# KushalChaudhari-16/Medical-Image-Denoising-Using-Diffusion

Measured on AMD Instinct MI355X. Metric: denoised images/sec, 256x256 x50 DDIM steps, higher is better.
Workload: dtype f32 (split-fp16 x3 MFMA, fp32 accumulate); 1 GPU; batch=8/GPU 256x256 grayscale, 50-iteration reverse loop (noise_steps=50, inference_steps=50), random-init 12.8M-param UNet (BASELINE.json configs[1]); batch_per_gpu=8, global_batch=8, parallelism=single, collective=none

## Files before the change

medical-image-denoising-using-diffusion_amd/csrc/conv1x1_f16x3_body.h:

```cpp
#if !defined(MIDD_CONV1_KERNEL) || !defined(MIDD_CONV1_PL)
#error "include from conv1x1_f16x3.hip with MIDD_CONV1_KERNEL and MIDD_CONV1_PL defined"
#endif

template <int MT, int NT, int ATT>
__global__ __launch_bounds__(256, ATT == ATT_PART_IN ? 2 : 3)
void MIDD_CONV1_KERNEL(const ConvArgs a) {
    constexpr int PL = MIDD_CONV1_PL;
    static_assert(PL == 1 || PL == 2, "planes");
    using G = Conv1Geom<MT, NT, PL>;
    constexpr int BM = G::BM, WSTEP = G::WSTEP, WTILE = PL * 1024;
    extern __shared__ __attribute__((aligned(16))) char lds[];

    const int tid = threadIdx.x;
    const int lane = tid & 63;
    const int wave = __builtin_amdgcn_readfirstlane(tid >> 6);
    const int p16 = lane & 15;
    const int kq = lane >> 4;

    const int Cin = a.C0 + a.C1;
    const int csteps = (Cin + 31) >> 5;
    const int nsteps = csteps;
    const int HW = a.OH * a.OW;
    const int tiles = a.tiles_x;
    const int b = blockIdx.x / a.wgs_per_img;
    const int first_tile = blockIdx.x - b * a.wgs_per_img;
    const int my_tiles = (tiles - first_tile + a.wgs_per_img - 1) / a.wgs_per_img;
    const int ntiles_total = a.Cout >> 4;
    const int ntile_wg = blockIdx.y * NT;

    char* const wl = lds;
    float* const stat_lds = reinterpret_cast<float*>(wl + max(csteps * WSTEP, 4096));
    float* const add_lds = stat_lds + G::STAT_FLOATS;
    float* const gnp = add_lds + G::ADD_FLOATS;
    float* const coef_lds = gnp + 2 * Cin + 16;

    constexpr int SG = (ATT == ATT_PART_IN) ? 4 : 1;
    const size_t img0 = (size_t)b * HW;
    const size_t split_stride = (size_t)a.B * HW * Cin;
    auto load_a = [&](int tile, int step, f32x4 (&r)[SG][MT][2]) {
        const float* src; int cs;
        int ch = step * 32 + kq * 8;
        if (ch >= Cin) ch = Cin - 8;
        size_t pstride;
        if constexpr (ATT == ATT_PART_IN) {
            src = a.src0 + ch + img0 * Cin; pstride = (size_t)Cin; cs = Cin;
        } else {
            int nb, cc;
            if (ch < a.C0) { src = a.src0; nb = a.C0 >> 4; cc = ch; } else { src = a.src1; nb = a.C1 >> 4; cc = ch - a.C0; }
            src += ((size_t)(b * nb + (cc >> 4)) * HW) * 16 + (cc & 15); pstride = 16; cs = 0;
        }
        (void)cs;
#pragma unroll
        for (int mt = 0; mt < MT; ++mt) {
            const int p = min(tile * BM + (wave * MT + mt) * 16 + p16, HW - 1);
            const float* q = src + (size_t)p * pstride;
#pragma unroll
            for (int g = 0; g < SG; ++g) {
                const float* qg = q + (size_t)min(g, (ATT == ATT_PART_IN ? a.att_ksplit : 1) - 1) * split_stride;
                r[g][mt][0] = *reinterpret_cast<const f32x4*>(qg);
                r[g][mt][1] = *reinterpret_cast<const f32x4*>(qg + 4);
            }
        }
    };
    f32x4 ra[2][SG][MT][2];
    const int total = my_tiles * nsteps;
    int pf_tile = first_tile, pf_step = 0;
    auto advance = [&](int& tile, int& step) { if (++step == nsteps) { step = 0; tile += a.wgs_per_img; } };
    load_a(pf_tile, pf_step, ra[0]); advance(pf_tile, pf_step);
    if (total > 1) { load_a(pf_tile, pf_step, ra[1]); advance(pf_tile, pf_step); }

    {
        const char* wbase = reinterpret_cast<const char*>(a.wpack) + (size_t)ntile_wg * WTILE + lane * 16;
        const size_t wstep_bytes = (size_t)ntiles_total * WTILE;
        const int pieces = csteps * NT * PL;
        for (int piece = wave; piece < pieces; piece += G::NW) {
            const int step = piece / (NT * PL), r = piece - step * (NT * PL);
            dma16(wbase + step * wstep_bytes + r * 1024, wl + piece * 1024);
        }
    }
    if (a.prologue != PRO_RAW)
        gn_prologue_lds(a.gn_tot0, a.C0, a.gn_bs0, a.gn_tot1, a.C1, a.gn_bs1, a.stat_rep, a.gn_gamma, a.gn_beta, a.gn_eps, a.gn_inv_n, b, ACT_PRESCALE, gnp, tid, G::NTHREADS, a.status);
    stat_word* const raw_acc = reinterpret_cast<stat_word*>(gnp);
    if (a.prologue == PRO_RAW && a.gn_tot0 != nullptr && wave == 0)
        raw_sumsq_lds(a.gn_tot0, a.C0, a.gn_bs0, a.gn_tot1, a.C1, a.gn_bs1, a.stat_rep, b, raw_acc, lane);
    {
        const int trow = (a.temb != nullptr) ? a.trow[b] : 0;
        for (int i = tid; i < G::ADD_FLOATS; i += G::NTHREADS) {
            const int co = ntile_wg * 16 + i;
            add_lds[i] = a.bias[co] + (a.temb != nullptr ? a.temb[(size_t)trow * a.temb_stride + co] : 0.f);
        }
    }
    float rscale = a.raw_scale_fixed, oscale = a.out_scale;
    auto tile_coef = [&](int tile, bool sync) {
        if constexpr (ATT == ATT_PART_IN) {
            if (sync) lds_barrier();
            const int heads = a.att_heads, ks = a.att_ksplit;
            for (int i = tid; i < BM * heads; i += G::NTHREADS) {
                const int head = i / BM, pix = i - head * BM;
                const int p = min(tile * BM + pix, HW - 1);
                const float* ml0 = a.att_ml + (((size_t)b * heads + head) * HW + p) * 2;
                const size_t ml_stride = (size_t)a.B * heads * HW * 2;
                float mv[C1_MAX_SPLIT], lv[C1_MAX_SPLIT];
                float M = -INFINITY;
#pragma unroll
                for (int sp = 0; sp < C1_MAX_SPLIT; ++sp) {
                    mv[sp] = -INFINITY; lv[sp] = 0.f;
                    if (sp < ks) { mv[sp] = ml0[sp * ml_stride]; lv[sp] = ml0[sp * ml_stride + 1]; }
                    M = fmaxf(M, mv[sp]);
                }
                float L = 0.f;
#pragma unroll
                for (int sp = 0; sp < C1_MAX_SPLIT; ++sp) { mv[sp] = __builtin_amdgcn_exp2f(mv[sp] - M); L += lv[sp] * mv[sp]; }
                const float inv = rscale / (L * 16384.0f);
#pragma unroll
                for (int sp = 0; sp < C1_MAX_SPLIT; ++sp) coef_lds[(sp * heads + head) * BM + pix] = mv[sp] * inv;
            }
            if (sync) lds_barrier();
        }
    };

    if constexpr (ATT == ATT_PART_IN) tile_coef(first_tile, false);
    asm volatile("s_waitcnt vmcnt(0) lgkmcnt(0)" ::: "memory");
    __builtin_amdgcn_s_barrier();
    asm volatile("" ::: "memory");
    if (a.prologue == PRO_RAW) {
        if (a.gn_tot0 != nullptr) {
            bool bad;
            const int ex = __builtin_amdgcn_readfirstlane(raw_prescale_exp(raw_acc, &bad));
            rscale = pow2f(ex);
            if (bad && tid == 0 && a.status != nullptr) atomicOr(a.status, (int)STATUS_NONFINITE);
        }
        oscale = a.out_scale / rscale;
    }

    f32x4 acc[MT][NT];
#pragma unroll
    for (int mt = 0; mt < MT; ++mt)
#pragma unroll
        for (int nt = 0; nt < NT; ++nt) acc[mt][nt] = (f32x4){0.f, 0.f, 0.f, 0.f};

    const int ntile0 = ntile_wg;
    f32x4 ssum[NT], ssq[NT];
#pragma unroll
    for (int nt = 0; nt < NT; ++nt) { ssum[nt] = (f32x4){0.f, 0.f, 0.f, 0.f}; ssq[nt] = (f32x4){0.f, 0.f, 0.f, 0.f}; }
    typedef unsigned u32x2 __attribute__((ext_vector_type(2)));
    auto epilogue = [&](int tile) {
#pragma unroll
        for (int nt = 0; nt < NT; ++nt) {
            const int co = (ntile0 + nt) * 16 + kq * 4;
            const f32x4 add = *reinterpret_cast<const f32x4*>(add_lds + nt * 16 + kq * 4);
            if constexpr (ATT == ATT_QKV_OUT) {
                const int C = a.att_heads * a.att_D;
                const int co0 = (ntile0 + nt) * 16;
                const int part = co0 / C, cc0 = co0 - part * C;
                const int head = cc0 / a.att_D, d = cc0 - head * a.att_D + kq * 4;
#pragma unroll
                for (int mt = 0; mt < MT; ++mt) {
                    const int p = tile * BM + (wave * MT + mt) * 16 + p16;
                    f32x4 v = acc[mt][nt] * oscale + add;
                    if (part == 0) {
                        if (p < HW) *reinterpret_cast<f32x4*>(a.out + (img0 + p) * C + cc0 + kq * 4) = v;
                    } else if (p < a.att_npad) {
                        if (p >= HW) v = (f32x4){0.f, 0.f, 0.f, 0.f};
                        const float big = fmaxf(fmaxf(fabsf(v[0]), fabsf(v[1])), fmaxf(fabsf(v[2]), fabsf(v[3])));
                        if (!(big < 65504.0f / ACT_PRESCALE) && a.status != nullptr) atomicOr(a.status, (int)STATUS_FP16_RANGE);
                        unsigned h01, h23, l01, l23;
                        planes_pair<PL>(v[0] * ACT_PRESCALE, v[1] * ACT_PRESCALE, h01, l01);
                        planes_pair<PL>(v[2] * ACT_PRESCALE, v[3] * ACT_PRESCALE, h23, l23);
                        _Float16* img = (part == 1 ? a.att_k : a.att_v) + ((size_t)(b * a.att_heads + head) * PL) * a.att_npad * a.att_D;
                        *reinterpret_cast<u32x2*>(img + (size_t)p * a.att_D + d) = (u32x2){h01, h23};
                        if constexpr (PL == 2) *reinterpret_cast<u32x2*>(img + (size_t)(a.att_npad + p) * a.att_D + d) = (u32x2){l01, l23};
                    }
                    acc[mt][nt] = (f32x4){0.f, 0.f, 0.f, 0.f};
                }
            } else {
#pragma unroll
                for (int mt = 0; mt < MT; ++mt) {
                    const int p = tile * BM + (wave * MT + mt) * 16 + p16;
                    if (p < HW) {
                        const size_t o = (((size_t)b * (a.Cout >> 4) + (co >> 4)) * HW + p) * 16 + (co & 15);
                        f32x4 v = acc[mt][nt] * oscale + add;
                        if (a.resid != nullptr) v += *reinterpret_cast<const f32x4*>(a.resid + o);
                        *reinterpret_cast<f32x4*>(a.out + o) = v;
                        ssum[nt] += v; ssq[nt] += v * v;
                    }
                    acc[mt][nt] = (f32x4){0.f, 0.f, 0.f, 0.f};
                }
            }
        }
    };

    int c_tile = first_tile, c_step = 0;
    auto compute = [&](f32x4 (&r)[SG][MT][2], bool more) {
        const int cstep = c_step;
        if constexpr (ATT == ATT_PART_IN) {
            if (c_step == 0 && c_tile != first_tile) tile_coef(c_tile, true);
        }
        const int ch = cstep * 32 + kq * 8;
        const bool valid = ch < Cin;
        f32x4 sc0 = {rscale, rscale, rscale, rscale}, sc1 = sc0;
        f32x4 sh0 = {0.f, 0.f, 0.f, 0.f}, sh1 = sh0;
        if (a.prologue != PRO_RAW && valid) {
            sc0 = *reinterpret_cast<const f32x4*>(gnp + ch);       sc1 = *reinterpret_cast<const f32x4*>(gnp + ch + 4);
            sh0 = *reinterpret_cast<const f32x4*>(gnp + Cin + ch); sh1 = *reinterpret_cast<const f32x4*>(gnp + Cin + ch + 4);
        }
        half8 xh[MT], xl[MT];
#pragma unroll
        for (int mt = 0; mt < MT; ++mt) {
            f32x4 v0, v1;
            if constexpr (ATT == ATT_PART_IN) {
                const float* cf = coef_lds + (ch / a.att_D) * BM + (wave * MT + mt) * 16 + p16;
                const int cstride = a.att_heads * BM;
                v0 = (f32x4){0.f, 0.f, 0.f, 0.f}; v1 = v0;
#pragma unroll
                for (int g = 0; g < SG; ++g) { const float c = cf[g * cstride]; v0 += r[g][mt][0] * c; v1 += r[g][mt][1] * c; }
                for (int g0 = SG; g0 < a.att_ksplit; g0 += SG) {
                    f32x4 t[SG][2];
                    const int p = min(c_tile * BM + (wave * MT + mt) * 16 + p16, HW - 1);
                    const float* q = a.src0 + ch + (img0 + p) * Cin;
#pragma unroll
                    for (int g = 0; g < SG; ++g) {
                        const float* qg = q + (size_t)min(g0 + g, a.att_ksplit - 1) * split_stride;
                        t[g][0] = *reinterpret_cast<const f32x4*>(qg); t[g][1] = *reinterpret_cast<const f32x4*>(qg + 4);
                    }
#pragma unroll
                    for (int g = 0; g < SG; ++g) { const float c = cf[(g0 + g) * cstride]; v0 += t[g][0] * c; v1 += t[g][1] * c; }
                }
            } else {
                v0 = r[0][mt][0] * sc0 + sh0; v1 = r[0][mt][1] * sc1 + sh1;
            }
            if (a.prologue == PRO_GN_SILU) {
#pragma unroll
                for (int e = 0; e < 4; ++e) {
                    v0[e] = v0[e] * __builtin_amdgcn_rcpf(1.0f + __builtin_amdgcn_exp2f(v0[e] * (-1.4426950408889634f / ACT_PRESCALE)));
                    v1[e] = v1[e] * __builtin_amdgcn_rcpf(1.0f + __builtin_amdgcn_exp2f(v1[e] * (-1.4426950408889634f / ACT_PRESCALE)));
                }
            }
            if (!valid) { v0 = (f32x4){0.f, 0.f, 0.f, 0.f}; v1 = v0; }
            typedef unsigned u32x4 __attribute__((ext_vector_type(4)));
            u32x4 hw, lw;
            unsigned hh, ll;
            planes_pair<PL>(v0[0], v0[1], hh, ll); hw[0] = hh; lw[0] = ll;
            planes_pair<PL>(v0[2], v0[3], hh, ll); hw[1] = hh; lw[1] = ll;
            planes_pair<PL>(v1[0], v1[1], hh, ll); hw[2] = hh; lw[2] = ll;
            planes_pair<PL>(v1[2], v1[3], hh, ll); hw[3] = hh; lw[3] = ll;
            xh[mt] = __builtin_bit_cast(half8, hw);
            xl[mt] = __builtin_bit_cast(half8, lw);
        }
        if (more) { load_a(pf_tile, pf_step, r); advance(pf_tile, pf_step); }
        const char* wslot = wl + cstep * WSTEP + lane * 16;
        half8 wh[NT], wlo[NT];
#pragma unroll
        for (int nt = 0; nt < NT; ++nt) {
            wh[nt] = *reinterpret_cast<const half8*>(wslot + nt * WTILE);
            if constexpr (PL == 2) wlo[nt] = *reinterpret_cast<const half8*>(wslot + nt * WTILE + 1024);
        }
#pragma unroll
        for (int mt = 0; mt < MT; ++mt)
#pragma unroll
            for (int nt = 0; nt < NT; ++nt)
                acc[mt][nt] = __builtin_amdgcn_mfma_f32_16x16x32_f16(wh[nt], xh[mt], acc[mt][nt], 0, 0, 0);
        if constexpr (PL == 2) {
#pragma unroll
            for (int mt = 0; mt < MT; ++mt)
#pragma unroll
                for (int nt = 0; nt < NT; ++nt)
                    acc[mt][nt] = __builtin_amdgcn_mfma_f32_16x16x32_f16(wh[nt], xl[mt], acc[mt][nt], 0, 0, 0);
#pragma unroll
            for (int mt = 0; mt < MT; ++mt)
#pragma unroll
                for (int nt = 0; nt < NT; ++nt)
                    acc[mt][nt] = __builtin_amdgcn_mfma_f32_16x16x32_f16(wlo[nt], xh[mt], acc[mt][nt], 0, 0, 0);
        }
        if (c_step == nsteps - 1) epilogue(c_tile);
        advance(c_tile, c_step);
    };
    for (int s = 0; s < total; s += 2) {
        compute(ra[0], s + 2 < total);
        if (s + 1 < total) compute(ra[1], s + 3 < total);
    }

    if (a.stat_tot != nullptr) {
        float* const my_stat = stat_lds + wave * (2 * NT * 16) + kq * 4;
#pragma unroll
        for (int nt = 0; nt < NT; ++nt) {
#pragma unroll
            for (int e = 0; e < 4; ++e) { ssum[nt][e] = row16_sum(ssum[nt][e]); ssq[nt][e] = row16_sum(ssq[nt][e]); }
            if (p16 == 0) {
                lds_store_raw(my_stat + nt * 16, ssum[nt]);
                lds_store_raw(my_stat + NT * 16 + nt * 16, ssq[nt]);
            }
        }
        constexpr int ROWF = 2 * NT * 16;
        asm volatile("s_waitcnt lgkmcnt(0)" ::: "memory");
        __builtin_amdgcn_s_barrier();
        asm volatile("" ::: "memory");
        auto fold = [&](int i) {
            float t = 0.f;
#pragma unroll
            for (int m = 0; m < G::NW; ++m) t += stat_lds[m * ROWF + i];
            return t;
        };
        stat_publish(a.stat_tot, b, a.Cout, a.stat_bs, a.stat_rep, first_tile % a.stat_rep, ntile_wg * 16, NT * 16,
                     fold, reinterpret_cast<stat_word*>(wl), tid, G::NTHREADS);
    }
}
```

medical-image-denoising-using-diffusion_amd/csrc/conv_mfma_f16x3_body.h:

```cpp
#if !defined(MIDD_CONV16_KERNEL) || !defined(MIDD_CONV16_PL)
#error "include from conv_mfma_f16x3.hip with MIDD_CONV16_KERNEL and MIDD_CONV16_PL defined"
#endif

template <int KS, int STRIDE, int TW, int MT, int NT, int WM, int WN, bool RES, int CBT>
__global__ MIDD_CONV16_BOUNDS void MIDD_CONV16_KERNEL(const ConvArgs a) {
    constexpr int PL = MIDD_CONV16_PL;
    static_assert(PL == 1 || PL == 2, "planes");
    using G = Conv16Geom<KS, STRIDE, TW, MT, NT, WM, WN, CBT, PL>;
    constexpr int NW = G::NW, NTHREADS = G::NTHREADS, TH = G::TH, IW = G::IW;
    constexpr int PAD = (KS == 3) ? 1 : 0;
    constexpr int NSLOT = G::NSLOT, APW = G::APW, PLANE = G::PLANE;
    constexpr int TAPS = KS * KS;
    constexpr int HSTEPS = (TAPS + 1) / 2;
    constexpr int PPW = G::PPW, WSLICE = G::WSLICE, RING = G::RING;

    extern __shared__ __attribute__((aligned(16))) char lds[];
    char* const raw = lds;
    char* const img = lds + G::RAW_BYTES;
    char* const wring = img + G::IMG_BYTES;
    float* const stat_lds = reinterpret_cast<float*>(wring + RING * WSLICE);
    float* const add_lds = stat_lds + G::STAT_FLOATS;
    float* const gnp = add_lds + G::ADD_FLOATS;

    const int tid = threadIdx.x;
// ... 30 lines not shown
    unsigned dma_bad = 0;
    auto sent4 = [](unsigned v) { typedef unsigned u32x4_ __attribute__((ext_vector_type(4))); return __builtin_bit_cast(f32x4, (u32x4_){v, v, v, v}); };
    auto has_sent = [](const auto& q, unsigned v) {
        typedef unsigned u32x4_ __attribute__((ext_vector_type(4)));
        const u32x4_ u = __builtin_bit_cast(u32x4_, q);
        return (unsigned)((u[0] == v) | (u[1] == v) | (u[2] == v) | (u[3] == v));
    };
#endif
    auto issue_w = [&]() {
        char* slot = wring + wr_slot * WSLICE;
#ifdef MIDD_DMA_CHECK
#pragma unroll
        for (int i = 0; i < PPW; ++i) {
            int piece = (WM == 1) ? wave * PPW + i : wave + i * NW;
            if (piece >= G::WPIECES) piece -= G::WPIECES;
            if constexpr (PL == 1) piece %= G::WPIECES;
            lds_store_raw(slot + piece * 1024 + lane16, sent4(SENT_W));
        }
        asm volatile("s_waitcnt lgkmcnt(0)" ::: "memory");
#endif
#pragma unroll
        for (int i = 0; i < PPW; ++i) {
            int piece = (WM == 1) ? wave * PPW + i : wave + i * NW;
            if (piece >= G::WPIECES) piece -= G::WPIECES;
            if constexpr (PL == 1) piece %= G::WPIECES;
            dma16(wr_src + piece * 1024 + lane16, slot + piece * 1024);
        }
        ++wr_step; wr_src += wstep_bytes;
        if (wr_step == total_steps) { wr_step = 0; wr_src = wbase; }
        wr_slot = (wr_slot + 1 == RING) ? 0 : wr_slot + 1;
    };

    const int q8 = tid % QPP;
    const int sblk = q8 >> 2;
    int g_off[APW];
    bool tile_pad = true;
    auto set_tile = [&](int t) {
        const int iy0 = (t / a.tiles_x) * TH * STRIDE - PAD, ix0 = (t % a.tiles_x) * TW * STRIDE - PAD;
        tile_pad = iy0 < 0 || ix0 < 0 || iy0 + G::IH > a.H || ix0 + IW > a.W;
        int tid_ = tid;
        asm volatile("" : "+v"(tid_));
#pragma unroll
        for (int s = 0; s < APW; ++s) {
            const int slot = tid_ + s * NTHREADS;
            int off = -2;
            if (slot < NSLOT) {
                const int pix = slot / QPP;
                const int iy = pix / IW, ix = pix - iy * IW;
                const int gy = iy0 + iy, gx = ix0 + ix;
                off = (gy >= 0 && gy < a.H && gx >= 0 && gx < a.W) ? gy * a.W + gx : -1;
            }
            g_off[s] = off;
        }
    };
    set_tile(trem);
    auto issue_a = [&](int c) {
        const int blk = min(CB * c + sblk, nblk - 1);
        const float* src; int bsrc, nb;
        if ((blk << 4) < a.C0) { src = a.src0; bsrc = blk; nb = a.C0 >> 4; }
        else                   { src = a.src1; bsrc = blk - (a.C0 >> 4); nb = a.C1 >> 4; }
        const char* base = reinterpret_cast<const char*>(src) + ((size_t)(b * nb + bsrc) * (size_t)(a.H * a.W)) * 64 + (q8 & 3) * 16;
#ifdef MIDD_DMA_CHECK
#pragma unroll
        for (int s = 0; s < APW; ++s) lds_store_raw(raw + (wave + s * NW) * 1024 + lane16, sent4(SENT_A));
        asm volatile("s_waitcnt lgkmcnt(0)" ::: "memory");
#endif
#pragma unroll
        for (int s = 0; s < APW; ++s) {
            const unsigned byte_off = (unsigned)max(g_off[s], 0) * 64u;
            dma16(base + byte_off, raw + (wave + s * NW) * 1024);
        }
    };
    float rscale = RAW_PRESCALE;
    auto transform = [&](int c) {
        const int blk = CB * c + sblk;
        if (blk >= nblk) return;
        const int ch = (blk << 4) + (q8 & 3) * 4;
        f32x4 rq[APW];
#pragma unroll
        for (int s = 0; s < APW; ++s) rq[s] = *reinterpret_cast<const f32x4*>(raw + (tid + s * NTHREADS) * 16);
#ifdef MIDD_DMA_CHECK
#pragma unroll
        for (int s = 0; s < APW; ++s) dma_bad |= has_sent(rq[s], SENT_A);
#endif
        f32x4 sc = {rscale, rscale, rscale, rscale}, sh = {0.f, 0.f, 0.f, 0.f};
        if (a.prologue != PRO_RAW) {
            sc = *reinterpret_cast<const f32x4*>(gnp + ch);
            sh = *reinterpret_cast<const f32x4*>(gnp + Cin + ch);
        }
        char* base = img + sblk * PL * PLANE + (q8 & 3) * 8;
        typedef unsigned u32x2 __attribute__((ext_vector_type(2)));
        if (c == 0 && tile_pad) {
#pragma unroll
            for (int s = 0; s < APW; ++s) {
                const int slot = tid + s * NTHREADS;
                if (g_off[s] == -1) {
                    *reinterpret_cast<u32x2*>(base + (slot / QPP) * 32) = (u32x2){0u, 0u};
                    if constexpr (PL == 2) *reinterpret_cast<u32x2*>(base + PLANE + (slot / QPP) * 32) = (u32x2){0u, 0u};
                }
            }
        }
#pragma unroll
        for (int s = 0; s < APW; ++s) {
            const int slot = tid + s * NTHREADS;
            float v[4];
#pragma unroll
            for (int e = 0; e < 4; ++e) v[e] = __builtin_fmaf(rq[s][e], sc[e], sh[e]);
#if defined(C16_ABL) && C16_ABL == 4
            if (false) {
#else
            if (a.prologue == PRO_GN_SILU) {
#endif
#pragma unroll
                for (int e = 0; e < 4; ++e) {
                    const float d = __builtin_fmaf(__builtin_amdgcn_exp2f(v[e]), 1.0f / ACT_PRESCALE, 1.0f / ACT_PRESCALE);
                    v[e] = v[e] * __builtin_amdgcn_rcpf(d);
                }
            }
            unsigned h01, h23, l01, l23;
            planes_pair<PL>(v[0], v[1], h01, l01);
            planes_pair<PL>(v[2], v[3], h23, l23);
            if (g_off[s] >= 0) {
                const int pix = slot / QPP;
                *reinterpret_cast<u32x2*>(base + pix * 32) = (u32x2){h01, h23};
                if constexpr (PL == 2) *reinterpret_cast<u32x2*>(base + PLANE + pix * 32) = (u32x2){l01, l23};
            }
        }
    };

    int frag_base[MT];
#pragma unroll
    for (int mt = 0; mt < MT; ++mt) {
        const int pp = (wm * MT + mt) * 16 + p16;
        const int py = pp / TW, px = pp - py * TW;
        frag_base[mt] = ((py * STRIDE) * IW + px * STRIDE) * 32 + (kq & 1) * 16;
    }
    int frag_full[MT];
#pragma unroll
    for (int mt = 0; mt < MT; ++mt) frag_full[mt] = frag_base[mt] + (kq >> 1) * PL * PLANE;
    const int wfrag_off = (wn * NT) * WTILE + lane * 16;

    f32x4 acc[MT][NT];
#pragma unroll
    for (int mt = 0; mt < MT; ++mt)
#pragma unroll
        for (int nt = 0; nt < NT; ++nt) acc[mt][nt] = (f32x4){0.f, 0.f, 0.f, 0.f};

    constexpr int D = RING - 1;
    constexpr bool PAIR = conv16_pair_walk(TAPS, CB);
    static_assert(D <= 5, "the chunk-end wait has one arm per after = 1 .. 4 below D (MIDD_RING_MAX 6)");
    constexpr auto cmin = [](int x, int y) { return x < y ? x : y; };
    const int ntile0 = ntile_wg + wn * NT;
    TS_DECL
    issue_a(0);
#pragma unroll
    for (int i = 0; i < D; ++i) issue_w();
#if !(defined(C16_ABL) && C16_ABL == 6)
    if (a.prologue == PRO_GN || a.prologue == PRO_GN_SILU)
        gn_prologue_lds(a.gn_tot0, a.C0, a.gn_bs0, a.gn_tot1, a.C1, a.gn_bs1, a.stat_rep, a.gn_gamma, a.gn_beta, a.gn_eps, a.gn_inv_n, b,
                        (a.prologue == PRO_GN_SILU) ? SILU_ARG_FACTOR : ACT_PRESCALE, gnp, tid, NTHREADS, a.status);
#endif
    stat_word* const raw_acc = reinterpret_cast<stat_word*>(gnp);
    if (a.prologue == PRO_RAW && a.gn_tot0 != nullptr && wave == 0)
        raw_sumsq_lds(a.gn_tot0, a.C0, a.gn_bs0, a.gn_tot1, a.C1, a.gn_bs1, a.stat_rep, b, raw_acc, lane);
    stat_word* const res_acc = reinterpret_cast<stat_word*>(gnp + 2 * Cin);
    if (res_steps > 0 && a.res_tot0 != nullptr && wave == NW - 1)
        raw_sumsq_lds(a.res_tot0, a.res_C0, a.res_bs0, a.res_tot1, a.res_C1, a.res_bs1, a.stat_rep, b, res_acc, lane);
    {
        const int trow = (a.temb != nullptr) ? a.trow[b] : 0;
        for (int i = tid; i < G::ADD_FLOATS; i += NTHREADS) {
            const int co = ntile_wg * 16 + i;
            add_lds[i] = a.bias[co] + (a.temb != nullptr ? a.temb[(size_t)trow * a.temb_stride + co] : 0.f);
        }
    }
    wait_vm_and_barrier<0>();
    float oscale = a.out_scale;
    if (a.prologue == PRO_RAW) {
        rscale = a.raw_scale_fixed;
        if (a.gn_tot0 != nullptr) {
            bool bad;
            const int ex = __builtin_amdgcn_readfirstlane(raw_prescale_exp(raw_acc, &bad));
            rscale = pow2f(ex);
            if (bad && tid == 0 && a.status != nullptr) atomicOr(a.status, (int)STATUS_NONFINITE);
        }
        oscale = a.out_scale / rscale;
    }
    float res_in = 1.0f, res_rescale = 1.0f;
    if (res_steps > 0) {
        if (a.res_tot0 != nullptr) {
            bool bad;
            res_in = pow2f(__builtin_amdgcn_readfirstlane(raw_prescale_exp(res_acc, &bad)));
            if (bad && tid == 0 && a.status != nullptr) atomicOr(a.status, (int)STATUS_NONFINITE);
        }
        res_rescale = a.out_scale * res_in / a.res_scale;
        oscale = a.res_scale / res_in;
    }
    transform(0);
    if constexpr (WM == 1) {
        asm volatile("s_waitcnt lgkmcnt(0)" ::: "memory");
        __builtin_amdgcn_s_barrier();
        asm volatile("" ::: "memory");
    }

    TS(TS_PROLOGUE)
    int frag_next[MT], frag_wrap[MT];
#pragma unroll
    for (int mt = 0; mt < MT; ++mt) {
        frag_next[mt] = frag_base[mt] + (kq >> 1) * 32;
        frag_wrap[mt] = frag_base[mt] + (kq >> 1) * ((IW - KS + 1) * 32);
    }
    int rd_slot = 0;
    half8 xh[MT], xl[MT];
    auto load_x = [&](const int (&xo)[MT], int off) {
#pragma unroll
        for (int mt = 0; mt < MT; ++mt) {
            xh[mt] = *reinterpret_cast<const half8*>(img + xo[mt] + off);
            if constexpr (PL == 2) xl[mt] = *reinterpret_cast<const half8*>(img + xo[mt] + off + PLANE);
        }
    };
    auto tap_off = [](int t) { return ((t / KS) * IW + (t % KS)) * 32; };
    auto kill_x = [&]() {
        if constexpr (PAIR) {
#pragma unroll
            for (int mt = 0; mt < MT; ++mt) {
                asm volatile("" : "=v"(xh[mt]));
                if constexpr (PL == 2) asm volatile("" : "=v"(xl[mt]));
            }
        }
    };
    auto load_stash = [&]() {
        constexpr int T8 = (((TAPS - 1) / KS) * IW + (TAPS - 1) % KS) * 32;
        if constexpr (MT == 2) {
            const int so = (kq >> 1) ? frag_base[1] : frag_base[0];
            xh[0] = *reinterpret_cast<const half8*>(img + so + T8);
            if constexpr (PL == 2) xl[0] = *reinterpret_cast<const half8*>(img + so + T8 + PLANE);
        } else {
            load_x(frag_base, T8);
        }
    };
    auto unpack_stash = [&]() {
        if constexpr (MT == 2) {
            typedef unsigned u32x4_ __attribute__((ext_vector_type(4)));
            auto unpack = [](half8& lo, half8& hi) {
                u32x4_ a = __builtin_bit_cast(u32x4_, lo), b = __builtin_bit_cast(u32x4_, hi);
#pragma unroll
                for (int r = 0; r < 4; ++r) {
                    const auto sw = __builtin_amdgcn_permlane32_swap(a[r], b[r], false, false);
                    a[r] = sw[0]; b[r] = sw[1];
                }
                lo = __builtin_bit_cast(half8, a); hi = __builtin_bit_cast(half8, b);
            };
            unpack(xh[0], xh[1]);
            if constexpr (PL == 2) unpack(xl[0], xl[1]);
        }
    };
    auto mfma_step = [&]() {
        const char* wslot = wring + rd_slot * WSLICE + wfrag_off;
        rd_slot = (rd_slot + 1 == RING) ? 0 : rd_slot + 1;
        half8 wh[NT], wl[NT];
#pragma unroll
        for (int nt = 0; nt < NT; ++nt) {
            wh[nt] = *reinterpret_cast<const half8*>(wslot + nt * WTILE);
            if constexpr (PL == 2) wl[nt] = *reinterpret_cast<const half8*>(wslot + nt * WTILE + 1024);
        }
#ifdef MIDD_DMA_CHECK
#pragma unroll
        for (int nt = 0; nt < NT; ++nt) {
            dma_bad |= has_sent(wh[nt], SENT_W);
            if constexpr (PL == 2) dma_bad |= has_sent(wl[nt], SENT_W);
        }
#endif
#pragma unroll
        for (int mt = 0; mt < MT; ++mt)
#pragma unroll
            for (int nt = 0; nt < NT; ++nt)
                acc[mt][nt] = __builtin_amdgcn_mfma_f32_16x16x32_f16(wh[nt], xh[mt], acc[mt][nt], 0, 0, 0);
#if !(defined(C16_ABL) && C16_ABL == 8)
        if constexpr (PL == 2) {
#pragma unroll
            for (int mt = 0; mt < MT; ++mt)
#pragma unroll
                for (int nt = 0; nt < NT; ++nt)
                    acc[mt][nt] = __builtin_amdgcn_mfma_f32_16x16x32_f16(wh[nt], xl[mt], acc[mt][nt], 0, 0, 0);
#pragma unroll
            for (int mt = 0; mt < MT; ++mt)
#pragma unroll
                for (int nt = 0; nt < NT; ++nt)
                    acc[mt][nt] = __builtin_amdgcn_mfma_f32_16x16x32_f16(wl[nt], xh[mt], acc[mt][nt], 0, 0, 0);
        }
#endif
    };

    auto k_step = [&](auto with_a, auto merge, bool first, bool first_with_more, int next_chunk, const int (&xo)[MT], int xoff) {
        constexpr bool WITH_A = decltype(with_a)::value;
        constexpr bool MERGE = decltype(merge)::value;
        auto load_frag = [&]() {
            if constexpr (MERGE) { unpack_stash(); if (kq >= 2) load_x(xo, xoff); }
            else load_x(xo, xoff);
        };
#ifdef MIDD_DMA_CHECK_BREAK
        constexpr int N = D * PPW + (WITH_A ? APW : 0);
#else
        constexpr int N = (D - 1) * PPW + (WITH_A ? APW : 0);
#endif
        const bool early = (WM == 1) || !first;
        if (early) {
            if constexpr (PL == 1) __builtin_amdgcn_sched_barrier(0);
            load_frag();
            asm volatile("s_waitcnt vmcnt(%0) lgkmcnt(%1)" ::"n"(N), "n"(PL * MT) : "memory");
        } else {
            asm volatile("s_waitcnt vmcnt(%0) lgkmcnt(0)" ::"n"(N) : "memory");
        }
        TS(TS_DMAWAIT)
        if constexpr (WM != 1) {
            __builtin_amdgcn_s_barrier();
            asm volatile("" ::: "memory");
        }
#ifdef MIDD_CONV_TIMING
        if (ts_after_epi) { TS(TS_FIRSTWAIT) ts_after_epi = false; } else { TS(TS_WAIT) }
#endif
        if (!early) load_frag();
        issue_w();
        if (first_with_more) issue_a(next_chunk);
        TS(TS_ISSUE)
        mfma_step();
        TS(TS_MFMA)
    };

    constexpr int RL = 2 * MT;
    constexpr int RG = (MT == 1) ? 2 : 1;
    static_assert((D - 1) * PPW + APW <= 63 && D * PPW <= 63 && (D - 1) * PPW + RG * RL <= 63 && RG * PPW <= 63, "vmcnt immediate beyond 63");
    auto res_load = [&](int r, f32x4 (&dst)[MT][2]) {
        const int rc = a.res_C0 + a.res_C1;
        int ch = r * 32 + kq * 8;
        if (ch >= rc) ch = rc - 8;
        const float* src; int nb, cc;
        if (ch < a.res_C0) { src = a.res_src0; nb = a.res_C0 >> 4; cc = ch; } else { src = a.res_src1; nb = a.res_C1 >> 4; cc = ch - a.res_C0; }
        src += ((size_t)(b * nb + (cc >> 4)) * (size_t)(a.OH * a.OW)) * 16 + (cc & 15);
#pragma unroll
        for (int mt = 0; mt < MT; ++mt) {
            const int pp = (wm * MT + mt) * 16 + p16;
            const int py = pp / TW, px = pp - py * TW;
            const int oy = min(oy0 + py, a.OH - 1), ox = min(ox0 + px, a.OW - 1);
            const float* q = src + (size_t)(oy * a.OW + ox) * 16;
#ifdef MIDD_DMA_CHECK
            dst[mt][0] = sent4(SENT_A); dst[mt][1] = sent4(SENT_A);
            asm volatile("global_load_dwordx4 %0, %1, off" : "+v"(dst[mt][0]) : "v"(q) : "memory");
            asm volatile("global_load_dwordx4 %0, %1, off offset:16" : "+v"(dst[mt][1]) : "v"(q) : "memory");
#else
// ... 290 lines not shown
```

medical-image-denoising-using-diffusion_amd/csrc/stats_common.h:

```cpp
#pragma once
#include <hip/hip_runtime.h>

namespace midd {

constexpr int GN_GROUPS_C = 8;
constexpr int STAT_LIMBS = 3;
constexpr int STAT_WORDS = 2 * STAT_LIMBS;
constexpr int STAT_MAX_REPLICAS = 8;
typedef unsigned long long stat_word;

__device__ __forceinline__ float stat_rstd(double var_plus_eps) {
    const float x = (float)var_plus_eps;
    float y = __builtin_amdgcn_rsqf(x);
    y = y * (1.5f - 0.5f * x * y * y);
    return y;
}

constexpr unsigned long long STAT_NAN_SENTINEL = 1ull << 50;
constexpr long long STAT_NAN_THRESHOLD = 1ll << 49;

__device__ __forceinline__ double stat_total(const stat_word* limbs) {
    const long long l0 = (long long)limbs[0], l1 = (long long)limbs[1], l2 = (long long)limbs[2];
    if (l2 >= STAT_NAN_THRESHOLD || l2 <= -STAT_NAN_THRESHOLD) return __builtin_nan("");
    return (double)l0 * 0x1p-60 + (double)l1 * 0x1p-20 + (double)l2 * 0x1p20;
}

__device__ __forceinline__ int stat_gcd(int a, int b) { while (b) { const int t = a % b; a = b; b = t; } return a; }

__device__ __forceinline__ void gn_prologue_lds(const stat_word* __restrict__ tot0, int C0, int bs0,
                                                const stat_word* __restrict__ tot1, int C1, int bs1, int rep,
                                                const float* __restrict__ gamma, const float* __restrict__ beta, float eps,
                                                double inv_n, int b, float mult, float* gnp, int tid, int nthreads, int* status = nullptr) {
    typedef unsigned long long u64x2 __attribute__((ext_vector_type(2)));
    const int Cin = C0 + C1, cg = Cin / GN_GROUPS_C;
    const int nb0 = C0 / bs0, nb1 = (C1 > 0) ? C1 / bs1 : 0;
    for (int c = tid; c < Cin; c += nthreads) {
        const float ga = gamma[c], be = beta[c];
        const int g = c / cg;
        stat_word acc[STAT_WORDS];
#pragma unroll
        for (int i = 0; i < STAT_WORDS; ++i) acc[i] = 0;
        int ch = g * cg;
        const int ch_end = ch + cg;
        while (ch < ch_end) {
            const stat_word* p;
            if (ch < C0) { p = tot0 + ((size_t)b * nb0 + ch / bs0) * rep * STAT_WORDS; ch += bs0; }
            else         { p = tot1 + ((size_t)b * nb1 + (ch - C0) / bs1) * rep * STAT_WORDS; ch += bs1; }
            for (int r = 0; r < rep; ++r) {
#pragma unroll
                for (int i = 0; i < STAT_WORDS; i += 2) {
                    const u64x2 v = *reinterpret_cast<const u64x2*>(p + r * STAT_WORDS + i);
                    acc[i] += v[0]; acc[i + 1] += v[1];
                }
            }
        }
        const double mean = stat_total(acc) * inv_n;
        double var = stat_total(acc + STAT_LIMBS) * inv_n - mean * mean;
        if (var < 0) var = 0;
        const float sc = stat_rstd(var + (double)eps) * ga;
        if (status != nullptr && !(mean == mean && var == var)) atomicOr(status, 1);
        gnp[c] = mult * sc;
        gnp[Cin + c] = mult * (be - (float)mean * sc);
    }
}

__device__ __forceinline__ unsigned lds_offset(const void* p) {
    return (unsigned)(unsigned long long)(const __attribute__((address_space(3))) char*)p;
}
__device__ __forceinline__ void lds_store_raw(void* p, float v) { asm volatile("ds_write_b32 %0, %1" ::"v"(lds_offset(p)), "v"(v) : "memory"); }
__device__ __forceinline__ void lds_store_raw(void* p, unsigned long long v) { asm volatile("ds_write_b64 %0, %1" ::"v"(lds_offset(p)), "v"(v) : "memory"); }
__device__ __forceinline__ void lds_store_raw(void* p, float __attribute__((ext_vector_type(4))) v) {
    asm volatile("ds_write_b128 %0, %1" ::"v"(lds_offset(p)), "v"(v) : "memory");
}
__device__ __forceinline__ void lds_add_raw(unsigned long long* p, unsigned long long v) { asm volatile("ds_add_u64 %0, %1" ::"v"(lds_offset(p)), "v"(v) : "memory"); }
__device__ __forceinline__ void lds_barrier_raw() {
    asm volatile("s_waitcnt lgkmcnt(0)" ::: "memory");
    __builtin_amdgcn_s_barrier();
    asm volatile("" ::: "memory");
}

__device__ __forceinline__ void stat_add_lds(stat_word* slot, float t) {
    const unsigned u = __float_as_uint(t);
    const int ex = (int)((u >> 23) & 0xffu);
    if (ex == 0) return;
    unsigned long long m = (unsigned long long)((u & 0x7fffffu) | 0x800000u);
    int s = ex - 150 + 60;
    if (ex == 255 || s > 95) { lds_add_raw(slot + 2, STAT_NAN_SENTINEL); return; }
    if (s < 0) { m = (s > -24) ? (m >> (-s)) : 0ull; s = 0; }
    const int k = s / 40, r = s - k * 40;
    const unsigned long long x = m << r;
    unsigned long long lo = x & ((1ull << 40) - 1ull), hi = x >> 40;
    if (u >> 31) { lo = 0ull - lo; hi = 0ull - hi; }
    if (lo) lds_add_raw(slot + k, lo);
    if (hi) lds_add_raw(slot + k + 1, hi);
}

__device__ __forceinline__ void raw_sumsq_lds(const stat_word* __restrict__ tot0, int C0, int bs0,
                                              const stat_word* __restrict__ tot1, int C1, int bs1, int rep, int b,
                                              stat_word* acc3, int lane) {
    if (lane < STAT_LIMBS) lds_store_raw(acc3 + lane, 0ull);
    const int nb0 = C0 / bs0, nb1 = (C1 > 0) ? C1 / bs1 : 0;
    for (int e = lane; e < (nb0 + nb1) * rep; e += 64) {
        const int blk = e / rep, r = e - blk * rep;
        const stat_word* p = (blk < nb0) ? tot0 + (((size_t)b * nb0 + blk) * rep + r) * STAT_WORDS
                                         : tot1 + (((size_t)b * nb1 + (blk - nb0)) * rep + r) * STAT_WORDS;
#pragma unroll
        for (int i = 0; i < STAT_LIMBS; ++i) {
            const stat_word v = p[STAT_LIMBS + i];
            if (v) lds_add_raw(acc3 + i, v);
        }
    }
}
__device__ __forceinline__ int raw_prescale_exp(const stat_word* acc3, bool* bad) {
    const float S = (float)stat_total(acc3);
    *bad = !(S < __builtin_inff());
    if (!(S > 0.f) || *bad) return 0;
    const int e = (int)((__float_as_uint(S) >> 23) & 0xffu) - 126;
    int a = 15 - ((e + 1) >> 1);
    if (a > 60) a = 60;
    return a;
}
__device__ __forceinline__ float pow2f(int a) { return __uint_as_float((unsigned)(127 + a) << 23); }

template <class Fold>
__device__ __forceinline__ void stat_publish(stat_word* __restrict__ tot, int b, int C, int bs, int rep, int replica,
                                             int c0, int ncol, Fold fold, stat_word* lds_acc, int tid, int nthreads) {
    const int blk_first = c0 / bs, nblk = (c0 + ncol - 1) / bs - blk_first + 1;
    for (int j = tid; j < nblk * STAT_WORDS; j += nthreads) lds_store_raw(lds_acc + j, 0ull);
    lds_barrier_raw();
    for (int i = tid; i < 2 * ncol; i += nthreads) {
        const int which = i / ncol, c = c0 + i - which * ncol;
        stat_add_lds(lds_acc + ((c / bs - blk_first) * 2 + which) * STAT_LIMBS, fold(i));
    }
    lds_barrier_raw();
    for (int j = tid; j < nblk * STAT_WORDS; j += nthreads) {
        const stat_word v = lds_acc[j];
#if defined(C16_ABL) && C16_ABL == 7
        if (v) tot[(((size_t)b * (C / bs) + blk_first + j / STAT_WORDS) * rep + replica) * STAT_WORDS + j % STAT_WORDS] = v;
#else
        if (v) atomicAdd(tot + (((size_t)b * (C / bs) + blk_first + j / STAT_WORDS) * rep + replica) * STAT_WORDS + j % STAT_WORDS, v);
#endif
    }
}

}
```

Baseline: 50.33 images/s.

## Parallelize GroupNorm stat gathering and overlap prologue loads with weight DMA

Reworks the conv kernel prologues. GroupNorm group statistics are now reduced across all threads into shared LDS group accumulators, replacing the single-wave raw_sumsq and the old gn_prologue path. Gamma/beta, bias/temb and the first tile's attention coefficients are loaded into registers before the weight-DMA barrier and written to LDS afterwards, so their global latency overlaps the weight and activation prefetch. This adds LDS atomics, an extra barrier, more register pressure, and reuses stat/image LDS regions for the accumulators.

```diff
diff --git a/medical-image-denoising-using-diffusion_amd/csrc/conv1x1_f16x3_body.h b/medical-image-denoising-using-diffusion_amd/csrc/conv1x1_f16x3_body.h
--- a/medical-image-denoising-using-diffusion_amd/csrc/conv1x1_f16x3_body.h
+++ b/medical-image-denoising-using-diffusion_amd/csrc/conv1x1_f16x3_body.h
@@ -62,6 +62,11 @@
             }
         }
     };
+    const int trow = (a.temb != nullptr) ? *(const __attribute__((address_space(4))) int*)(a.trow + b) : 0;
+    stat_word* const tot_acc = reinterpret_cast<stat_word*>(stat_lds);
+    static_assert(G::STAT_FLOATS * 4 >= TOT_ACC_WORDS * 8, "group accumulators in the output statistics' rows");
+    constexpr bool HAS_TOT = ATT != ATT_PART_IN;
+    if constexpr (HAS_TOT) tot_acc_zero(tot_acc, tid);
     f32x4 ra[2][SG][MT][2];
     const int total = my_tiles * nsteps;
     int pf_tile = first_tile, pf_step = 0;
@@ -78,53 +83,109 @@
             dma16(wbase + step * wstep_bytes + r * 1024, wl + piece * 1024);
         }
     }
-    if (a.prologue != PRO_RAW)
-        gn_prologue_lds(a.gn_tot0, a.C0, a.gn_bs0, a.gn_tot1, a.C1, a.gn_bs1, a.stat_rep, a.gn_gamma, a.gn_beta, a.gn_eps, a.gn_inv_n, b, ACT_PRESCALE, gnp, tid, G::NTHREADS, a.status);
-    stat_word* const raw_acc = reinterpret_cast<stat_word*>(gnp);
-    if (a.prologue == PRO_RAW && a.gn_tot0 != nullptr && wave == 0)
-        raw_sumsq_lds(a.gn_tot0, a.C0, a.gn_bs0, a.gn_tot1, a.C1, a.gn_bs1, a.stat_rep, b, raw_acc, lane);
-    {
-        const int trow = (a.temb != nullptr) ? a.trow[b] : 0;
-        for (int i = tid; i < G::ADD_FLOATS; i += G::NTHREADS) {
-            const int co = ntile_wg * 16 + i;
-            add_lds[i] = a.bias[co] + (a.temb != nullptr ? a.temb[(size_t)trow * a.temb_stride + co] : 0.f);
-        }
+    const bool gn = HAS_TOT && a.prologue != PRO_RAW;
+    constexpr int GNK = 2;
+    float ga[GNK], be[GNK];
+#pragma unroll
+    for (int k = 0; k < GNK; ++k) {
+        const int c = tid + k * G::NTHREADS;
+        ga[k] = 0.f; be[k] = 0.f;
+        if (gn && c < Cin) { ga[k] = a.gn_gamma[c]; be[k] = a.gn_beta[c]; }
+    }
+    static_assert(G::ADD_FLOATS <= G::NTHREADS, "one bias element per thread");
+    float addv = 0.f, tembv = 0.f;
+    if (tid < G::ADD_FLOATS) {
+        const int co = ntile_wg * 16 + tid;
+        addv = a.bias[co];
+        if (a.temb != nullptr) tembv = a.temb[(size_t)trow * a.temb_stride + co];
     }
     float rscale = a.raw_scale_fixed, oscale = a.out_scale;
-    auto tile_coef = [&](int tile, bool sync) {
+    auto coef_load = [&](int tile, int i, float (&mv)[C1_MAX_SPLIT], float (&lv)[C1_MAX_SPLIT]) {
+        const int heads = a.att_heads, ks = a.att_ksplit;
+        const int head = i / BM, pix = i - head * BM;
+        const int p = min(tile * BM + pix, HW - 1);
+        const float* ml0 = a.att_ml + (((size_t)b * heads + head) * HW + p) * 2;
+        const size_t ml_stride = (size_t)a.B * heads * HW * 2;
+#pragma unroll
+        for (int sp = 0; sp < C1_MAX_SPLIT; ++sp) {
+            mv[sp] = -INFINITY; lv[sp] = 0.f;
+            if (sp < ks) { mv[sp] = ml0[sp * ml_stride]; lv[sp] = ml0[sp * ml_stride + 1]; }
+        }
+    };
+    auto coef_store = [&](int i, float (&mv)[C1_MAX_SPLIT], float (&lv)[C1_MAX_SPLIT]) {
+        const int heads = a.att_heads;
+        const int head = i / BM, pix = i - head * BM;
+        float M = -INFINITY;
+#pragma unroll
+        for (int sp = 0; sp < C1_MAX_SPLIT; ++sp) M = fmaxf(M, mv[sp]);
+        float L = 0.f;
+#pragma unroll
+        for (int sp = 0; sp < C1_MAX_SPLIT; ++sp) { mv[sp] = __builtin_amdgcn_exp2f(mv[sp] - M); L += lv[sp] * mv[sp]; }
+        const float inv = rscale / (L * 16384.0f);
+#pragma unroll
+        for (int sp = 0; sp < C1_MAX_SPLIT; ++sp) coef_lds[(sp * heads + head) * BM + pix] = mv[sp] * inv;
+    };
+    auto tile_coef = [&](int tile) {
         if constexpr (ATT == ATT_PART_IN) {
-            if (sync) lds_barrier();
-            const int heads = a.att_heads, ks = a.att_ksplit;
-            for (int i = tid; i < BM * heads; i += G::NTHREADS) {
-                const int head = i / BM, pix = i - head * BM;
-                const int p = min(tile * BM + pix, HW - 1);
-                const float* ml0 = a.att_ml + (((size_t)b * heads + head) * HW + p) * 2;
-                const size_t ml_stride = (size_t)a.B * heads * HW * 2;
+            lds_barrier();
+            for (int i = tid; i < BM * a.att_heads; i += G::NTHREADS) {
                 float mv[C1_MAX_SPLIT], lv[C1_MAX_SPLIT];
-                float M = -INFINITY;
-#pragma unroll
-                for (int sp = 0; sp < C1_MAX_SPLIT; ++sp) {
-                    mv[sp] = -INFINITY; lv[sp] = 0.f;
-                    if (sp < ks) { mv[sp] = ml0[sp * ml_stride]; lv[sp] = ml0[sp * ml_stride + 1]; }
-                    M = fmaxf(M, mv[sp]);
-                }
-                float L = 0.f;
-#pragma unroll
-                for (int sp = 0; sp < C1_MAX_SPLIT; ++sp) { mv[sp] = __builtin_amdgcn_exp2f(mv[sp] - M); L += lv[sp] * mv[sp]; }
-                const float inv = rscale / (L * 16384.0f);
-#pragma unroll
-                for (int sp = 0; sp < C1_MAX_SPLIT; ++sp) coef_lds[(sp * heads + head) * BM + pix] = mv[sp] * inv;
-            }
-            if (sync) lds_barrier();
-        }
-    };
-
-    if constexpr (ATT == ATT_PART_IN) tile_coef(first_tile, false);
+                coef_load(tile, i, mv, lv);
+                coef_store(i, mv, lv);
+            }
+            lds_barrier();
+        }
+    };
+    float mv0[C1_MAX_SPLIT], lv0[C1_MAX_SPLIT];
+    constexpr bool COEF_EARLY = ATT == ATT_PART_IN && MT == 1;
+    if constexpr (COEF_EARLY) { if (tid < BM * a.att_heads) coef_load(first_tile, tid, mv0, lv0); }
+
+    const int cg = Cin / GN_GROUPS_C;
+    if constexpr (HAS_TOT) {
+        const int nb0 = a.C0 / a.gn_bs0, nb1 = (a.C1 > 0) ? a.C1 / a.gn_bs1 : 0;
+        const int nhalf = (a.gn_tot0 != nullptr) ? 2 * (nb0 + nb1) * a.stat_rep : 0;
+        auto half_rec = [&](int e, stat_word (&v)[STAT_LIMBS]) {
+            int ch, which;
+            const stat_word* p = tot_half(a.gn_tot0, a.C0, a.gn_bs0, nb0, a.gn_tot1, a.gn_bs1, nb1, a.stat_rep, b, e, &ch, &which);
+#pragma unroll
+            for (int i = 0; i < STAT_LIMBS; ++i) v[i] = p[i];
+            return (gn ? ch / cg : 0) * STAT_WORDS + which * STAT_LIMBS;
+        };
+        stat_word tq[STAT_LIMBS] = {0ull, 0ull, 0ull};
+        int tq_at = 0;
+        if (tid < nhalf) tq_at = half_rec(tid, tq);
+        lds_barrier_raw();
+        tot_add(tot_acc + tq_at, tq);
+        for (int e = tid + G::NTHREADS; e < nhalf; e += G::NTHREADS) {
+            stat_word v[STAT_LIMBS];
+            const int at = half_rec(e, v);
+            tot_add(tot_acc + at, v);
+        }
+    }
     asm volatile("s_waitcnt vmcnt(0) lgkmcnt(0)" ::: "memory");
     __builtin_amdgcn_s_barrier();
     asm volatile("" ::: "memory");
+    if (gn) {
+#pragma unroll
+        for (int k = 0; k < GNK; ++k) {
+            const int c = tid + k * G::NTHREADS;
+            if (c < Cin) gn_scale_shift_lds(tot_acc + (c / cg) * STAT_WORDS, ga[k], be[k], a.gn_eps, a.gn_inv_n, ACT_PRESCALE, gnp, Cin, c, a.status);
+        }
+        for (int c = tid + GNK * G::NTHREADS; c < Cin; c += G::NTHREADS)
+            gn_scale_shift_lds(tot_acc + (c / cg) * STAT_WORDS, a.gn_gamma[c], a.gn_beta[c], a.gn_eps, a.gn_inv_n, ACT_PRESCALE, gnp, Cin, c, a.status);
+    }
+    if (tid < G::ADD_FLOATS) add_lds[tid] = addv + tembv;
+    if constexpr (ATT == ATT_PART_IN) {
+        if constexpr (COEF_EARLY) { if (tid < BM * a.att_heads) coef_store(tid, mv0, lv0); }
+        for (int i = tid + (COEF_EARLY ? G::NTHREADS : 0); i < BM * a.att_heads; i += G::NTHREADS) {
+            float mv[C1_MAX_SPLIT], lv[C1_MAX_SPLIT];
+            coef_load(first_tile, i, mv, lv);
+            coef_store(i, mv, lv);
+        }
+    }
+    const stat_word* const raw_acc = tot_acc + STAT_LIMBS;
     if (a.prologue == PRO_RAW) {
-        if (a.gn_tot0 != nullptr) {
+        if (HAS_TOT && a.gn_tot0 != nullptr) {
             bool bad;
             const int ex = __builtin_amdgcn_readfirstlane(raw_prescale_exp(raw_acc, &bad));
             rscale = pow2f(ex);
@@ -132,6 +193,7 @@
         }
         oscale = a.out_scale / rscale;
     }
+    lds_barrier_raw();
 
     f32x4 acc[MT][NT];
 #pragma unroll
@@ -194,7 +256,7 @@
     auto compute = [&](f32x4 (&r)[SG][MT][2], bool more) {
         const int cstep = c_step;
         if constexpr (ATT == ATT_PART_IN) {
-            if (c_step == 0 && c_tile != first_tile) tile_coef(c_tile, true);
+            if (c_step == 0 && c_tile != first_tile) tile_coef(c_tile);
         }
         const int ch = cstep * 32 + kq * 8;
         const bool valid = ch < Cin;
diff --git a/medical-image-denoising-using-diffusion_amd/csrc/conv_mfma_f16x3_body.h b/medical-image-denoising-using-diffusion_amd/csrc/conv_mfma_f16x3_body.h
--- a/medical-image-denoising-using-diffusion_amd/csrc/conv_mfma_f16x3_body.h
+++ b/medical-image-denoising-using-diffusion_amd/csrc/conv_mfma_f16x3_body.h
@@ -206,28 +206,91 @@
     constexpr auto cmin = [](int x, int y) { return x < y ? x : y; };
     const int ntile0 = ntile_wg + wn * NT;
     TS_DECL
+    const int trow = (a.temb != nullptr) ? *(const __attribute__((address_space(4))) int*)(a.trow + b) : 0;
+    constexpr bool ACC_IN_IMG = G::STAT_FLOATS * 4 < TOT_ACC_WORDS * 8;
+    stat_word* const tot_acc = reinterpret_cast<stat_word*>(ACC_IN_IMG ? img : reinterpret_cast<char*>(stat_lds));
+    static_assert(G::IMG_BYTES >= TOT_ACC_WORDS * 8, "group accumulators in the MFMA image");
+    tot_acc_zero(tot_acc, tid);
     issue_a(0);
 #pragma unroll
     for (int i = 0; i < D; ++i) issue_w();
+    const bool gn = a.prologue == PRO_GN || a.prologue == PRO_GN_SILU;
+    const bool res_tot = RES && res_steps > 0 && a.res_tot0 != nullptr;
+    const int rnb0 = res_tot ? a.res_C0 / a.res_bs0 : 0, rnb1 = (res_tot && a.res_C1 > 0) ? a.res_C1 / a.res_bs1 : 0;
+    const int nres = (rnb0 + rnb1) * a.stat_rep;
+    stat_word rq[STAT_LIMBS] = {0ull, 0ull, 0ull};
+    auto res_rec = [&](int e) {
+        int ch, which;
+        const stat_word* p = tot_half(a.res_tot0, a.res_C0, a.res_bs0, rnb0, a.res_tot1, a.res_bs1, rnb1, a.stat_rep, b, 2 * e + 1, &ch, &which);
+#pragma unroll
+        for (int i = 0; i < STAT_LIMBS; ++i) rq[i] = p[i];
+    };
+    auto res_add = [&]() { tot_add(tot_acc + GN_GROUPS_C * STAT_WORDS + STAT_LIMBS, rq); };
+    if constexpr (RES) { if (tid < nres) res_rec(tid); }
+    constexpr int GNK = 2;
+    float ga[GNK], be[GNK];
+#pragma unroll
+    for (int k = 0; k < GNK; ++k) {
+        const int c = tid + k * NTHREADS;
+        ga[k] = 0.f; be[k] = 0.f;
+        if (gn && c < Cin) { ga[k] = a.gn_gamma[c]; be[k] = a.gn_beta[c]; }
+    }
+    constexpr int ADDK = (G::ADD_FLOATS + NTHREADS - 1) / NTHREADS;
+    float addv[ADDK], tembv[ADDK];
+#pragma unroll
+    for (int k = 0; k < ADDK; ++k) {
+        const int i = tid + k * NTHREADS;
+        addv[k] = 0.f; tembv[k] = 0.f;
+        if (i < G::ADD_FLOATS) {
+            const int co = ntile_wg * 16 + i;
+            addv[k] = a.bias[co];
+            if (a.temb != nullptr) tembv[k] = a.temb[(size_t)trow * a.temb_stride + co];
+        }
+    }
+    const int cg = Cin / GN_GROUPS_C;
+    const int nb0 = a.C0 / a.gn_bs0, nb1 = (a.C1 > 0) ? a.C1 / a.gn_bs1 : 0;
+    const int nhalf = (a.gn_tot0 != nullptr) ? 2 * (nb0 + nb1) * a.stat_rep : 0;
+    auto half_rec = [&](int e, stat_word (&v)[STAT_LIMBS]) {
+        int ch, which;
+        const stat_word* p = tot_half(a.gn_tot0, a.C0, a.gn_bs0, nb0, a.gn_tot1, a.gn_bs1, nb1, a.stat_rep, b, e, &ch, &which);
+#pragma unroll
+        for (int i = 0; i < STAT_LIMBS; ++i) v[i] = p[i];
+        return (gn ? ch / cg : 0) * STAT_WORDS + which * STAT_LIMBS;
+    };
+    stat_word tq[STAT_LIMBS] = {0ull, 0ull, 0ull};
+    int tq_at = 0;
+    if (tid < nhalf) tq_at = half_rec(tid, tq);
+    lds_barrier_raw();
+    tot_add(tot_acc + tq_at, tq);
+    for (int e = tid + NTHREADS; e < nhalf; e += NTHREADS) {
+        stat_word v[STAT_LIMBS];
+        const int at = half_rec(e, v);
+        tot_add(tot_acc + at, v);
+    }
+    if constexpr (RES) {
+        res_add();
+        for (int e = tid + NTHREADS; e < nres; e += NTHREADS) { res_rec(e); res_add(); }
+    }
+    wait_vm_and_barrier<0>();
 #if !(defined(C16_ABL) && C16_ABL == 6)
-    if (a.prologue == PRO_GN || a.prologue == PRO_GN_SILU)
-        gn_prologue_lds(a.gn_tot0, a.C0, a.gn_bs0, a.gn_tot1, a.C1, a.gn_bs1, a.stat_rep, a.gn_gamma, a.gn_beta, a.gn_eps, a.gn_inv_n, b,
-                        (a.prologue == PRO_GN_SILU) ? SILU_ARG_FACTOR : ACT_PRESCALE, gnp, tid, NTHREADS, a.status);
-#endif
-    stat_word* const raw_acc = reinterpret_cast<stat_word*>(gnp);
-    if (a.prologue == PRO_RAW && a.gn_tot0 != nullptr && wave == 0)
-        raw_sumsq_lds(a.gn_tot0, a.C0, a.gn_bs0, a.gn_tot1, a.C1, a.gn_bs1, a.stat_rep, b, raw_acc, lane);
-    stat_word* const res_acc = reinterpret_cast<stat_word*>(gnp + 2 * Cin);
-    if (res_steps > 0 && a.res_tot0 != nullptr && wave == NW - 1)
-        raw_sumsq_lds(a.res_tot0, a.res_C0, a.res_bs0, a.res_tot1, a.res_C1, a.res_bs1, a.stat_rep, b, res_acc, lane);
-    {
-        const int trow = (a.temb != nullptr) ? a.trow[b] : 0;
-        for (int i = tid; i < G::ADD_FLOATS; i += NTHREADS) {
-            const int co = ntile_wg * 16 + i;
-            add_lds[i] = a.bias[co] + (a.temb != nullptr ? a.temb[(size_t)trow * a.temb_stride + co] : 0.f);
-        }
-    }
-    wait_vm_and_barrier<0>();
+    if (gn) {
+        const float mult = (a.prologue == PRO_GN_SILU) ? SILU_ARG_FACTOR : ACT_PRESCALE;
+#pragma unroll
+        for (int k = 0; k < GNK; ++k) {
+            const int c = tid + k * NTHREADS;
+            if (c < Cin) gn_scale_shift_lds(tot_acc + (c / cg) * STAT_WORDS, ga[k], be[k], a.gn_eps, a.gn_inv_n, mult, gnp, Cin, c, a.status);
+        }
+        for (int c = tid + GNK * NTHREADS; c < Cin; c += NTHREADS)
+            gn_scale_shift_lds(tot_acc + (c / cg) * STAT_WORDS, a.gn_gamma[c], a.gn_beta[c], a.gn_eps, a.gn_inv_n, mult, gnp, Cin, c, a.status);
+    }
+#endif
+#pragma unroll
+    for (int k = 0; k < ADDK; ++k) {
+        const int i = tid + k * NTHREADS;
+        if (i < G::ADD_FLOATS) add_lds[i] = addv[k] + tembv[k];
+    }
+    const stat_word* const raw_acc = tot_acc + STAT_LIMBS;
+    const stat_word* const res_acc = tot_acc + GN_GROUPS_C * STAT_WORDS + STAT_LIMBS;
     float oscale = a.out_scale;
     if (a.prologue == PRO_RAW) {
         rscale = a.raw_scale_fixed;
@@ -249,6 +312,7 @@
         res_rescale = a.out_scale * res_in / a.res_scale;
         oscale = a.res_scale / res_in;
     }
+    if (gn || ACC_IN_IMG) lds_barrier_raw();
     transform(0);
     if constexpr (WM == 1) {
         asm volatile("s_waitcnt lgkmcnt(0)" ::: "memory");
diff --git a/medical-image-denoising-using-diffusion_amd/csrc/stats_common.h b/medical-image-denoising-using-diffusion_amd/csrc/stats_common.h
--- a/medical-image-denoising-using-diffusion_amd/csrc/stats_common.h
+++ b/medical-image-denoising-using-diffusion_amd/csrc/stats_common.h
@@ -79,6 +79,39 @@
     asm volatile("" ::: "memory");
 }
 
+constexpr int TOT_ACC_SLOTS = GN_GROUPS_C + 1;
+constexpr int TOT_ACC_WORDS = TOT_ACC_SLOTS * STAT_WORDS;
+
+__device__ __forceinline__ void tot_acc_zero(stat_word* acc, int tid) { if (tid < TOT_ACC_WORDS) lds_store_raw(acc + tid, 0ull); }
+
+__device__ __forceinline__ const stat_word* tot_half(const stat_word* __restrict__ tot0, int C0, int bs0, int nb0,
+                                                     const stat_word* __restrict__ tot1, int bs1, int nb1, int rep, int b, int e,
+                                                     int* ch, int* which) {
+    const int rec = e >> 1, blk = rec / rep, r = rec - blk * rep;
+    *which = e & 1;
+    if (blk < nb0) { *ch = blk * bs0; return tot0 + (((size_t)b * nb0 + blk) * rep + r) * STAT_WORDS + (e & 1) * STAT_LIMBS; }
+    *ch = C0 + (blk - nb0) * bs1;
+    return tot1 + (((size_t)b * nb1 + (blk - nb0)) * rep + r) * STAT_WORDS + (e & 1) * STAT_LIMBS;
+}
+__device__ __forceinline__ void tot_add(stat_word* acc, const stat_word (&v)[STAT_LIMBS]) {
+#pragma unroll
+    for (int i = 0; i < STAT_LIMBS; ++i)
+        if (v[i]) lds_add_raw(acc + i, v[i]);
+}
+__device__ __forceinline__ void gn_scale_shift_lds(const stat_word* grp, float ga, float be, float eps, double inv_n, float mult,
+                                                   float* gnp, int Cin, int c, int* status) {
+    stat_word acc[STAT_WORDS];
+#pragma unroll
+    for (int i = 0; i < STAT_WORDS; ++i) acc[i] = grp[i];
+    const double mean = stat_total(acc) * inv_n;
+    double var = stat_total(acc + STAT_LIMBS) * inv_n - mean * mean;
+    if (var < 0) var = 0;
+    const float sc = stat_rstd(var + (double)eps) * ga;
+    if (status != nullptr && !(mean == mean && var == var)) atomicOr(status, 1);
+    gnp[c] = mult * sc;
+    gnp[Cin + c] = mult * (be - (float)mean * sc);
+}
+
 __device__ __forceinline__ void stat_add_lds(stat_word* slot, float t) {
     const unsigned u = __float_as_uint(t);
     const int ex = (int)((u >> 23) & 0xffu);
@@ -95,22 +128,6 @@
     if (hi) lds_add_raw(slot + k + 1, hi);
 }
 
-__device__ __forceinline__ void raw_sumsq_lds(const stat_word* __restrict__ tot0, int C0, int bs0,
-                                              const stat_word* __restrict__ tot1, int C1, int bs1, int rep, int b,
-                                              stat_word* acc3, int lane) {
-    if (lane < STAT_LIMBS) lds_store_raw(acc3 + lane, 0ull);
-    const int nb0 = C0 / bs0, nb1 = (C1 > 0) ? C1 / bs1 : 0;
-    for (int e = lane; e < (nb0 + nb1) * rep; e += 64) {
-        const int blk = e / rep, r = e - blk * rep;
-        const stat_word* p = (blk < nb0) ? tot0 + (((size_t)b * nb0 + blk) * rep + r) * STAT_WORDS
-                                         : tot1 + (((size_t)b * nb1 + (blk - nb0)) * rep + r) * STAT_WORDS;
-#pragma unroll
-        for (int i = 0; i < STAT_LIMBS; ++i) {
-            const stat_word v = p[STAT_LIMBS + i];
-            if (v) lds_add_raw(acc3 + i, v);
-        }
-    }
-}
 __device__ __forceinline__ int raw_prescale_exp(const stat_word* acc3, bool* bad) {
     const float S = (float)stat_total(acc3);
     *bad = !(S < __builtin_inff());
```

Result: no change. 50.52 images/s (median of 4 runs) (+0.4%).
